# hku-mars/Voxel-SLAM

Measured on AMD Instinct MI355X. Metric: BA iterations/sec (10-frame window, 100k pts/scan), higher is better.
Workload: dtype f64; 1 GPU; cfg2: W=10, 100000 pts/scan, 50000 voxels per GPU, nnz=500000; global_voxels=50000, parallelism=voxel-shard x1, ranks_seen=1, collectives_per_lm_step=0, allreduce_doubles=0, lm_steps_accepted=2028, lm_steps_rejected=0

## Files before the change

### voxel-slam_amd/csrc/vxba_solve4.hpp

```cpp
#pragma once

typedef double s4v2 __attribute__((ext_vector_type(2)));

constexpr int S4_WAVES = 4;
constexpr int S4_THREADS = 64 * S4_WAVES;
constexpr int S4_ROW = 6;
constexpr int S4_BLK = 64 * S4_ROW + 6;
constexpr int S4_GSLOT = 64 * S4_ROW;

template <int W>
struct S4 {
  static constexpr int N = 6 * W, M = N - 6, B = W - 1;
  static constexpr int TC = 0;
  static constexpr int G = TC + (B > 0 ? B : 1) * S4_BLK;
  static constexpr int BV = G + (B > 0 ? B : 1) * S4_GSLOT;
  static constexpr int ZV = BV + 64;
  static constexpr int XS = ZV + 64;
  static constexpr int DOUBLES = XS + 64;
};

__device__ __forceinline__ double s4_rcp(double d) {
  const double r = __builtin_amdgcn_rcp(d);
  const double e = fma(-d, r, 1.0);
  const double t = fma(e, e, e);
  const double q = fma(r, t, r);
  return fabs(d) > 1e-300 ? q : 0.0;
}

__device__ __forceinline__ void s4_ldl6(double (&D)[21], double (&inv)[6]) {
#pragma unroll
  for (int p = 0; p < 6; p++) {
    inv[p] = s4_rcp(D[p * (p + 1) / 2 + p]);
    double col[6];
#pragma unroll
    for (int q = p + 1; q < 6; q++) col[q] = D[q * (q + 1) / 2 + p];
#pragma unroll
    for (int q = p + 1; q < 6; q++) {
      const double l = col[q] * inv[p];
#pragma unroll
      for (int r = p + 1; r <= q; r++) D[q * (q + 1) / 2 + r] = fma(-l, col[r], D[q * (q + 1) / 2 + r]);
      D[q * (q + 1) / 2 + p] = l;
    }
  }
}

__device__ __forceinline__ void s4_load_row(const double* p, double (&a)[6]) {
  const s4v2* v = reinterpret_cast<const s4v2*>(p);
  const s4v2 t0 = v[0], t1 = v[1], t2 = v[2];
  a[0] = t0[0]; a[1] = t0[1]; a[2] = t1[0]; a[3] = t1[1]; a[4] = t2[0]; a[5] = t2[1];
}
__device__ __forceinline__ void s4_store_row(double* p, const double (&a)[6]) {
  s4v2* v = reinterpret_cast<s4v2*>(p);
  v[0] = (s4v2){a[0], a[1]};
  v[1] = (s4v2){a[2], a[3]};
  v[2] = (s4v2){a[4], a[5]};
}

template <int W>
__device__ __forceinline__ void s4_apply(const double* lds, int t, int b, int lane, double (&T)[6]) {
  using C = S4<W>;
  double g[6];
  s4_load_row(lds + C::G + t * S4_GSLOT + lane * S4_ROW, g);
  const double* lr = lds + C::TC + t * S4_BLK + (6 * b) * S4_ROW;
#pragma unroll
  for (int c = 0; c < 6; c++) {
    double l[6];
    s4_load_row(lr + c * S4_ROW, l);
#pragma unroll
    for (int p = 0; p < 6; p++) T[c] = fma(-g[p], l[p], T[c]);
  }
}

constexpr int li_rec_len(int W) { return 1 + 12 * W + 6 * W + 36 * W * W; }
constexpr int li_out_len(int W) { return 6 * W + 12 * W + 1; }
template <int W, bool DBG>
__device__ __forceinline__ int lm_solve_body4(LMState* st, int c, double* lds, const double* __restrict__ li_rec = nullptr, double* __restrict__ li_out = nullptr,
                                               unsigned li_seq = 0) {
  using C = S4<W>;
  LMCtl& ctl = st->ctl[c];
  const int loop_done = ctl.done;
  constexpr int n = C::N, M = C::M, B = C::B;
  const int tid = threadIdx.x, lane = tid & 63;
  const int wave = __builtin_amdgcn_readfirstlane(tid >> 6);
  dbg_stamp(DBG && wave == 0, 4000, 0);
  dbg_stamp(DBG && wave == 0, 4000, 1);
  const double u = li_rec ? li_rec[0] : ctl.u;
  const double* __restrict__ li_x = li_rec ? li_rec + 1 : nullptr;
  const double* __restrict__ li_e = li_rec ? li_rec + 1 + 12 * W : nullptr;
  const double* __restrict__ li_E = li_rec ? li_rec + 1 + 18 * W : nullptr;
  const bool row_ok = lane < M;
  const int gi_row = row_ok ? 6 + lane : 0;

  constexpr int NQ = (B + S4_WAVES - 1) / S4_WAVES;
  double a0[NQ > 0 ? NQ : 1][6];
#pragma unroll
  for (int q = 0; q < NQ; q++) {
    const int b = wave + S4_WAVES * q;
    const int bb = b < B ? b : 0;
#pragma unroll
    for (int cc = 0; cc < 6; cc++) {
      const int col = 6 + 6 * bb + cc;
      const double h = st->Hwork[(size_t)col * n + gi_row];
      const double add = (li_E && gi_row >= 6 + 6 * bb) ? li_E[(size_t)col * n + gi_row] : 0.0;
      a0[q][cc] = row_ok ? (((col == gi_row) ? h + u * h : h) + add) : 0.0;
    }
  }
  double hii = 0.0, gi = 0.0, rhs0 = 0.0;
  double xcur[12];
  if (wave == 0) {
    hii = st->Hwork[(size_t)gi_row * n + gi_row];
    gi = st->Jwork[gi_row];
    const int fl = lane < W ? lane : 0;
#pragma unroll
    for (int k = 0; k < 12; k++) xcur[k] = li_x ? li_x[12 * fl + k] : ctl.x[12 * fl + k];
  }
  if (wave == 1 % S4_WAVES) rhs0 = row_ok ? (li_e ? li_e[gi_row] : 0.0) - st->Jwork[gi_row] : 0.0;
  if (loop_done) return 1;
  if (wave < B) s4_store_row(lds + C::TC + wave * S4_BLK + lane * S4_ROW, a0[0]);
  dbg_stamp(DBG && wave == 0, 4000, 2);

  int ap0 = -1, ap1 = -1, ap2 = -1;
  for (int s = 0; s < B; s++) {
    const int owner = s & (S4_WAVES - 1);
    double Ld[21], inv[6], g[6];
    if (wave == owner) {
      const int sq = s >> 2;
      const int ap = sq == 0 ? ap0 : (sq == 1 ? ap1 : ap2);
      double* trow = lds + C::TC + s * S4_BLK + lane * S4_ROW;
      double a[6];
      dbg_stamp(DBG, 4010 + s, 0);
      s4_load_row(trow, a);
      for (int t = ap + 1; t < s; t++) s4_apply<W>(lds, t, s, lane, a);
      if (DBG) { asm volatile("" :: "v"(a[0]), "v"(a[5])); dbg_stamp(true, 4010 + s, 1); }
      s4_store_row(trow, a);
      __builtin_amdgcn_wave_barrier();
      {
        const double* dr = lds + C::TC + s * S4_BLK + (6 * s) * S4_ROW;
        const s4v2 r0 = *reinterpret_cast<const s4v2*>(dr);
        const s4v2 r1 = *reinterpret_cast<const s4v2*>(dr + 6);
        const s4v2 r2a = *reinterpret_cast<const s4v2*>(dr + 12), r2b = *reinterpret_cast<const s4v2*>(dr + 14);
        const s4v2 r3a = *reinterpret_cast<const s4v2*>(dr + 18), r3b = *reinterpret_cast<const s4v2*>(dr + 20);
        const s4v2 r4a = *reinterpret_cast<const s4v2*>(dr + 24), r4b = *reinterpret_cast<const s4v2*>(dr + 26), r4c = *reinterpret_cast<const s4v2*>(dr + 28);
        const s4v2 r5a = *reinterpret_cast<const s4v2*>(dr + 30), r5b = *reinterpret_cast<const s4v2*>(dr + 32), r5c = *reinterpret_cast<const s4v2*>(dr + 34);
        Ld[0] = r0[0];
        Ld[1] = r1[0]; Ld[2] = r1[1];
        Ld[3] = r2a[0]; Ld[4] = r2a[1]; Ld[5] = r2b[0];
        Ld[6] = r3a[0]; Ld[7] = r3a[1]; Ld[8] = r3b[0]; Ld[9] = r3b[1];
        Ld[10] = r4a[0]; Ld[11] = r4a[1]; Ld[12] = r4b[0]; Ld[13] = r4b[1]; Ld[14] = r4c[0];
        Ld[15] = r5a[0]; Ld[16] = r5a[1]; Ld[17] = r5b[0]; Ld[18] = r5b[1]; Ld[19] = r5c[0]; Ld[20] = r5c[1];
      }
      if (DBG) { asm volatile("" :: "v"(Ld[0]), "v"(Ld[20])); dbg_stamp(true, 4010 + s, 2); }
      s4_ldl6(Ld, inv);
      if (DBG) { asm volatile("" :: "v"(inv[5])); dbg_stamp(true, 4010 + s, 3); }
      double l[6];
#pragma unroll
      for (int p = 0; p < 6; p++) {
        double acc = a[p];
#pragma unroll
        for (int q = 0; q < p; q++) acc = fma(-g[q], Ld[p * (p + 1) / 2 + q], acc);
        g[p] = acc;
        l[p] = acc * inv[p];
      }
      s4_store_row(trow, l);
      s4_store_row(lds + C::G + s * S4_GSLOT + lane * S4_ROW, g);
      if (sq == 0) ap0 = s; else if (sq == 1) ap1 = s; else ap2 = s;
      dbg_stamp(DBG, 4010 + s, 4);
    }
    if (s == 0) {
#pragma unroll
      for (int q = 1; q < NQ; q++) {
        const int b = wave + S4_WAVES * q;
        if (b < B) s4_store_row(lds + C::TC + b * S4_BLK + lane * S4_ROW, a0[q]);
      }
      if (wave == 1 % S4_WAVES) lds[C::BV + lane] = rhs0;
    }
    if (s < 9) dbg_stamp(DBG, 4000 + wave, 6 + 2 * s);
    __syncthreads();
    if (s < 9) dbg_stamp(DBG, 4000 + wave, 7 + 2 * s);
    if (wave == owner) {
      double bb[6];
      s4_load_row(lds + C::BV + 6 * s, bb);
      double br = lds[C::BV + lane];
      double z[6];
#pragma unroll
      for (int p = 0; p < 6; p++) {
        double acc = bb[p];
#pragma unroll
        for (int q = 0; q < p; q++) acc = fma(-bb[q], Ld[p * (p + 1) / 2 + q], acc);
        bb[p] = acc;
        z[p] = acc * inv[p];
      }
#pragma unroll
      for (int p = 0; p < 6; p++) br = fma(-g[p], z[p], br);
      const int d = lane - 6 * s;
      double zsel = z[0];
#pragma unroll
      for (int p = 1; p < 6; p++) zsel = (d == p) ? z[p] : zsel;
      if (d >= 0 && d < 6) lds[C::ZV + lane] = zsel;
      else lds[C::BV + lane] = br;
    }
    const bool next_owner = (s + 1 < B) && wave == ((s + 1) & (S4_WAVES - 1));
    if (!next_owner) {
      int budget = 2;
#pragma unroll
      for (int q = 0; q < (B + S4_WAVES - 1) / S4_WAVES; q++) {
        const int b = wave + S4_WAVES * q;
        int ap = q == 0 ? ap0 : (q == 1 ? ap1 : ap2);
        const bool must = b == s + 2;
        if (b > s && b < B && ap < s && (must || budget > 0)) {
          double* trow = lds + C::TC + b * S4_BLK + lane * S4_ROW;
          double T[6];
          s4_load_row(trow, T);
          while (ap < s && (must || budget > 0)) {
            s4_apply<W>(lds, ap + 1, b, lane, T);
            ap++;
            budget--;
          }
          s4_store_row(trow, T);
          if (q == 0) ap0 = ap; else if (q == 1) ap1 = ap; else ap2 = ap;
        }
      }
    }
  }
  __syncthreads();
  dbg_stamp(DBG && wave == 0, 4000, 3);
  if (wave != 0) return 0;

  double x = row_ok ? lds[C::ZV + lane] : 0.0;
  if constexpr (B > 0) {
    const int jb = (row_ok ? lane : 0) / 6, jc = (row_ok ? lane : 0) % 6;
    const double* lcol = lds + C::TC + jb * S4_BLK + jc;
    double Lr[6], Ln[6];
#pragma unroll
    for (int k = 0; k < 6; k++) Lr[k] = lcol[(M - 1 - k) * S4_ROW];
    for (int rb = B - 1; rb >= 0; rb--) {
      if (rb > 0) {
#pragma unroll
        for (int k = 0; k < 6; k++) Ln[k] = lcol[(6 * rb - 1 - k) * S4_ROW];
      }
#pragma unroll
      for (int k = 0; k < 6; k++) {
        const int r = 6 * rb + 5 - k;
        const double xr = readlane_f64(x, r);
        x = (lane < r) ? fma(-Lr[k], xr, x) : x;
      }
#pragma unroll
      for (int k = 0; k < 6; k++) Lr[k] = Ln[k];
    }
  }
  dbg_stamp(DBG, 4000, 4);
  if (row_ok) st->dxi[6 + lane] = x;
  if (lane < 6) st->dxi[lane] = 0.0;
  double* xs = lds + C::XS;
  if (lane < 6) xs[lane] = 0.0;
  if (row_ok) xs[6 + lane] = x;
  __builtin_amdgcn_wave_barrier();
  if (lane < W) {
    double dl[6];
#pragma unroll
    for (int k = 0; k < 6; k++) dl[k] = xs[6 * lane + k];
    double xn[9];
    lm_right_multiply_exp(xcur, dl, xn);
#pragma unroll
    for (int k = 0; k < 9; k++) __hip_atomic_store(&ctl.xt[12 * lane + k], xn[k], __ATOMIC_RELAXED, __HIP_MEMORY_SCOPE_AGENT);
#pragma unroll
    for (int k = 0; k < 3; k++) __hip_atomic_store(&ctl.xt[12 * lane + 9 + k], xcur[9 + k] + dl[3 + k], __ATOMIC_RELAXED, __HIP_MEMORY_SCOPE_AGENT);
    if (li_out) {
#pragma unroll
      for (int k = 0; k < 9; k++) li_out[6 * W + 12 * lane + k] = xn[k];
#pragma unroll
      for (int k = 0; k < 3; k++) li_out[6 * W + 12 * lane + 9 + k] = xcur[9 + k] + dl[3 + k];
    }
  }
  if (li_out) {
    if (row_ok) li_out[6 + lane] = x;
    if (lane < 6) li_out[lane] = 0.0;
    asm volatile("s_waitcnt vmcnt(0)" ::: "memory");
    __builtin_amdgcn_wave_barrier();
    if (lane == 0) li_out[18 * W] = (double)li_seq;
  }
  double part = row_ok ? x * (u * hii * x - gi) : 0.0;
#pragma unroll
  for (int off = 32; off > 0; off >>= 1) part += __shfl_down(part, off);
  if (lane == 0) ctl.q1 = 0.5 * part;
  if (DBG) { asm volatile("s_waitcnt vmcnt(0)" ::: "memory"); dbg_stamp(true, 4000, 5); }
  return 0;
}
```

Before: 21240 iterations/s.

## Pin panel factorization to wave 0 and fold RHS into the factored panel

```diff
diff --git a/voxel-slam_amd/csrc/vxba_solve4.hpp b/voxel-slam_amd/csrc/vxba_solve4.hpp
--- a/voxel-slam_amd/csrc/vxba_solve4.hpp
+++ b/voxel-slam_amd/csrc/vxba_solve4.hpp
@@ -13,11 +13,10 @@
   static constexpr int N = 6 * W, M = N - 6, B = W - 1;
   static constexpr int TC = 0;
   static constexpr int G = TC + (B > 0 ? B : 1) * S4_BLK;
-  static constexpr int BV = G + (B > 0 ? B : 1) * S4_GSLOT;
-  static constexpr int ZV = BV + 64;
-  static constexpr int XS = ZV + 64;
+  static constexpr int XS = G + (B > 0 ? B : 1) * S4_GSLOT;
   static constexpr int DOUBLES = XS + 64;
 };
+static_assert(6 * 10 - 6 < 64, "the right-hand side is row M of the block columns: M < 64 lanes");
 
 __device__ __forceinline__ double s4_rcp(double d) {
   const double r = __builtin_amdgcn_rcp(d);
@@ -73,6 +72,7 @@
 
 constexpr int li_rec_len(int W) { return 1 + 12 * W + 6 * W + 36 * W * W; }
 constexpr int li_out_len(int W) { return 6 * W + 12 * W + 1; }
+constexpr int S4_HELPERS = S4_WAVES - 1;
 template <int W, bool DBG>
 __device__ __forceinline__ int lm_solve_body4(LMState* st, int c, double* lds, const double* __restrict__ li_rec = nullptr, double* __restrict__ li_out = nullptr,
                                                unsigned li_seq = 0) {
@@ -89,129 +89,100 @@
   const double* __restrict__ li_e = li_rec ? li_rec + 1 + 12 * W : nullptr;
   const double* __restrict__ li_E = li_rec ? li_rec + 1 + 18 * W : nullptr;
   const bool row_ok = lane < M;
+  const bool rhs_row = B > 0 && lane == M;
   const int gi_row = row_ok ? 6 + lane : 0;
 
-  constexpr int NQ = (B + S4_WAVES - 1) / S4_WAVES;
-  double a0[NQ > 0 ? NQ : 1][6];
-#pragma unroll
-  for (int q = 0; q < NQ; q++) {
-    const int b = wave + S4_WAVES * q;
-    const int bb = b < B ? b : 0;
+  auto load_col = [&](int b, double (&a)[6]) __attribute__((always_inline)) {
 #pragma unroll
     for (int cc = 0; cc < 6; cc++) {
-      const int col = 6 + 6 * bb + cc;
+      const int col = 6 + 6 * b + cc;
       const double h = st->Hwork[(size_t)col * n + gi_row];
-      const double add = (li_E && gi_row >= 6 + 6 * bb) ? li_E[(size_t)col * n + gi_row] : 0.0;
-      a0[q][cc] = row_ok ? (((col == gi_row) ? h + u * h : h) + add) : 0.0;
-    }
-  }
-  double hii = 0.0, gi = 0.0, rhs0 = 0.0;
+      const double add = (li_E && gi_row >= 6 + 6 * b) ? li_E[(size_t)col * n + gi_row] : 0.0;
+      const double r = rhs_row ? (li_e ? li_e[col] : 0.0) - st->Jwork[col] : 0.0;
+      a[cc] = row_ok ? (((col == gi_row) ? h + u * h : h) + add) : r;
+    }
+  };
+  constexpr int NQ = B > 1 ? (B - 1 + S4_HELPERS - 1) / S4_HELPERS : 1;
+  double A[6];
+  double a0[NQ][6];
+  double hii = 0.0, gi = 0.0;
   double xcur[12];
   if (wave == 0) {
+    load_col(0, A);
     hii = st->Hwork[(size_t)gi_row * n + gi_row];
     gi = st->Jwork[gi_row];
     const int fl = lane < W ? lane : 0;
 #pragma unroll
     for (int k = 0; k < 12; k++) xcur[k] = li_x ? li_x[12 * fl + k] : ctl.x[12 * fl + k];
-  }
-  if (wave == 1 % S4_WAVES) rhs0 = row_ok ? (li_e ? li_e[gi_row] : 0.0) - st->Jwork[gi_row] : 0.0;
+  } else {
+#pragma unroll
+    for (int q = 0; q < NQ; q++) {
+      const int b = 1 + (wave - 1) + S4_HELPERS * q;
+      load_col(b < B ? b : (B > 1 ? 1 : 0), a0[q]);
+    }
+  }
   if (loop_done) return 1;
-  if (wave < B) s4_store_row(lds + C::TC + wave * S4_BLK + lane * S4_ROW, a0[0]);
+  if (wave != 0) {
+#pragma unroll
+    for (int q = 0; q < NQ; q++) {
+      const int b = 1 + (wave - 1) + S4_HELPERS * q;
+      if (b < B) s4_store_row(lds + C::TC + b * S4_BLK + lane * S4_ROW, a0[q]);
+    }
+  }
   dbg_stamp(DBG && wave == 0, 4000, 2);
 
+  double gp[6], lp[6];
   int ap0 = -1, ap1 = -1, ap2 = -1;
   for (int s = 0; s < B; s++) {
-    const int owner = s & (S4_WAVES - 1);
-    double Ld[21], inv[6], g[6];
-    if (wave == owner) {
-      const int sq = s >> 2;
-      const int ap = sq == 0 ? ap0 : (sq == 1 ? ap1 : ap2);
-      double* trow = lds + C::TC + s * S4_BLK + lane * S4_ROW;
-      double a[6];
+    if (wave == 0) {
       dbg_stamp(DBG, 4010 + s, 0);
-      s4_load_row(trow, a);
-      for (int t = ap + 1; t < s; t++) s4_apply<W>(lds, t, s, lane, a);
-      if (DBG) { asm volatile("" :: "v"(a[0]), "v"(a[5])); dbg_stamp(true, 4010 + s, 1); }
-      s4_store_row(trow, a);
-      __builtin_amdgcn_wave_barrier();
-      {
-        const double* dr = lds + C::TC + s * S4_BLK + (6 * s) * S4_ROW;
-        const s4v2 r0 = *reinterpret_cast<const s4v2*>(dr);
-        const s4v2 r1 = *reinterpret_cast<const s4v2*>(dr + 6);
-        const s4v2 r2a = *reinterpret_cast<const s4v2*>(dr + 12), r2b = *reinterpret_cast<const s4v2*>(dr + 14);
-        const s4v2 r3a = *reinterpret_cast<const s4v2*>(dr + 18), r3b = *reinterpret_cast<const s4v2*>(dr + 20);
-        const s4v2 r4a = *reinterpret_cast<const s4v2*>(dr + 24), r4b = *reinterpret_cast<const s4v2*>(dr + 26), r4c = *reinterpret_cast<const s4v2*>(dr + 28);
-        const s4v2 r5a = *reinterpret_cast<const s4v2*>(dr + 30), r5b = *reinterpret_cast<const s4v2*>(dr + 32), r5c = *reinterpret_cast<const s4v2*>(dr + 34);
-        Ld[0] = r0[0];
-        Ld[1] = r1[0]; Ld[2] = r1[1];
-        Ld[3] = r2a[0]; Ld[4] = r2a[1]; Ld[5] = r2b[0];
-        Ld[6] = r3a[0]; Ld[7] = r3a[1]; Ld[8] = r3b[0]; Ld[9] = r3b[1];
-        Ld[10] = r4a[0]; Ld[11] = r4a[1]; Ld[12] = r4b[0]; Ld[13] = r4b[1]; Ld[14] = r4c[0];
-        Ld[15] = r5a[0]; Ld[16] = r5a[1]; Ld[17] = r5b[0]; Ld[18] = r5b[1]; Ld[19] = r5c[0]; Ld[20] = r5c[1];
+      if (s > 0) {
+        double T[6];
+        s4_load_row(lds + C::TC + s * S4_BLK + lane * S4_ROW, T);
+#pragma unroll
+        for (int cc = 0; cc < 6; cc++) {
+          double lr[6];
+#pragma unroll
+          for (int p = 0; p < 6; p++) lr[p] = readlane_f64(lp[p], 6 * s + cc);
+#pragma unroll
+          for (int p = 0; p < 6; p++) T[cc] = fma(-gp[p], lr[p], T[cc]);
+        }
+#pragma unroll
+        for (int k = 0; k < 6; k++) A[k] = T[k];
+      }
+      if (DBG) { asm volatile("" :: "v"(A[0]), "v"(A[5])); dbg_stamp(true, 4010 + s, 1); }
+      double Ld[21], inv[6];
+#pragma unroll
+      for (int q = 0; q < 6; q++) {
+#pragma unroll
+        for (int p = 0; p <= q; p++) Ld[q * (q + 1) / 2 + p] = readlane_f64(A[p], 6 * s + q);
       }
       if (DBG) { asm volatile("" :: "v"(Ld[0]), "v"(Ld[20])); dbg_stamp(true, 4010 + s, 2); }
       s4_ldl6(Ld, inv);
       if (DBG) { asm volatile("" :: "v"(inv[5])); dbg_stamp(true, 4010 + s, 3); }
-      double l[6];
 #pragma unroll
       for (int p = 0; p < 6; p++) {
-        double acc = a[p];
-#pragma unroll
-        for (int q = 0; q < p; q++) acc = fma(-g[q], Ld[p * (p + 1) / 2 + q], acc);
-        g[p] = acc;
-        l[p] = acc * inv[p];
-      }
-      s4_store_row(trow, l);
-      s4_store_row(lds + C::G + s * S4_GSLOT + lane * S4_ROW, g);
-      if (sq == 0) ap0 = s; else if (sq == 1) ap1 = s; else ap2 = s;
+        double acc = A[p];
+#pragma unroll
+        for (int q = 0; q < p; q++) acc = fma(-gp[q], Ld[p * (p + 1) / 2 + q], acc);
+        gp[p] = acc;
+        lp[p] = acc * inv[p];
+      }
+      s4_store_row(lds + C::TC + s * S4_BLK + lane * S4_ROW, lp);
+      s4_store_row(lds + C::G + s * S4_GSLOT + lane * S4_ROW, gp);
       dbg_stamp(DBG, 4010 + s, 4);
-    }
-    if (s == 0) {
-#pragma unroll
-      for (int q = 1; q < NQ; q++) {
-        const int b = wave + S4_WAVES * q;
-        if (b < B) s4_store_row(lds + C::TC + b * S4_BLK + lane * S4_ROW, a0[q]);
-      }
-      if (wave == 1 % S4_WAVES) lds[C::BV + lane] = rhs0;
-    }
-    if (s < 9) dbg_stamp(DBG, 4000 + wave, 6 + 2 * s);
-    __syncthreads();
-    if (s < 9) dbg_stamp(DBG, 4000 + wave, 7 + 2 * s);
-    if (wave == owner) {
-      double bb[6];
-      s4_load_row(lds + C::BV + 6 * s, bb);
-      double br = lds[C::BV + lane];
-      double z[6];
-#pragma unroll
-      for (int p = 0; p < 6; p++) {
-        double acc = bb[p];
-#pragma unroll
-        for (int q = 0; q < p; q++) acc = fma(-bb[q], Ld[p * (p + 1) / 2 + q], acc);
-        bb[p] = acc;
-        z[p] = acc * inv[p];
-      }
-#pragma unroll
-      for (int p = 0; p < 6; p++) br = fma(-g[p], z[p], br);
-      const int d = lane - 6 * s;
-      double zsel = z[0];
-#pragma unroll
-      for (int p = 1; p < 6; p++) zsel = (d == p) ? z[p] : zsel;
-      if (d >= 0 && d < 6) lds[C::ZV + lane] = zsel;
-      else lds[C::BV + lane] = br;
-    }
-    const bool next_owner = (s + 1 < B) && wave == ((s + 1) & (S4_WAVES - 1));
-    if (!next_owner) {
+    } else {
       int budget = 2;
 #pragma unroll
-      for (int q = 0; q < (B + S4_WAVES - 1) / S4_WAVES; q++) {
-        const int b = wave + S4_WAVES * q;
+      for (int q = 0; q < NQ; q++) {
+        const int b = 1 + (wave - 1) + S4_HELPERS * q;
         int ap = q == 0 ? ap0 : (q == 1 ? ap1 : ap2);
-        const bool must = b == s + 2;
-        if (b > s && b < B && ap < s && (must || budget > 0)) {
+        const bool must = b == s + 1;
+        if (b > s && b < B && ap < s - 1 && (must || budget > 0)) {
           double* trow = lds + C::TC + b * S4_BLK + lane * S4_ROW;
           double T[6];
           s4_load_row(trow, T);
-          while (ap < s && (must || budget > 0)) {
+          while (ap < s - 1 && (must || budget > 0)) {
             s4_apply<W>(lds, ap + 1, b, lane, T);
             ap++;
             budget--;
@@ -221,15 +192,20 @@
         }
       }
     }
-  }
-  __syncthreads();
-  dbg_stamp(DBG && wave == 0, 4000, 3);
+    if (s + 1 < B) {
+      if (s < 9) dbg_stamp(DBG, 4000 + wave, 6 + 2 * s);
+      __syncthreads();
+      if (s < 9) dbg_stamp(DBG, 4000 + wave, 7 + 2 * s);
+    }
+  }
   if (wave != 0) return 0;
-
-  double x = row_ok ? lds[C::ZV + lane] : 0.0;
+  dbg_stamp(DBG, 4000, 3);
+
+  double x = 0.0;
   if constexpr (B > 0) {
     const int jb = (row_ok ? lane : 0) / 6, jc = (row_ok ? lane : 0) % 6;
     const double* lcol = lds + C::TC + jb * S4_BLK + jc;
+    x = row_ok ? lcol[M * S4_ROW] : 0.0;
     double Lr[6], Ln[6];
 #pragma unroll
     for (int k = 0; k < 6; k++) Lr[k] = lcol[(M - 1 - k) * S4_ROW];
```

New measurement: 18480 iterations/s (median of 2 runs). 0.87x the previous value.
